# FifthEpoch/longcat-video-tta

Measured on AMD Instinct MI355X. Metric: denoised latent frames/sec (49x720p, 50-step CFG denoise), higher is better.
Workload: dtype bf16; 1 GPU; K3: 49x720p (13 latent frames, 46 800 tokens); DiT 48 blocks x 4096 hidden, CFG 4.0, 50-step flow-match Euler, no conditioning frames; depth=48, parallelism=dp1

## Files before the change

### longcat-video-tta_amd/csrc/elementwise.hip

```cpp
#include "lcv_common.h"

#define ROWNORM_MAXCH 8

template <int MODE>
__global__ __launch_bounds__(256) void rownorm_fwd_kernel(
    const bf16_t* __restrict__ x, const float* __restrict__ p_add, const float* __restrict__ p_mul,
    bf16_t* __restrict__ y, int64_t rows, int C, int64_t S, int64_t mod_stride, float eps) {
  const int lane = threadIdx.x & 63;
  const int64_t row = (int64_t)blockIdx.x * 4 + (threadIdx.x >> 6);
  if (row >= rows) return;
  const bf16_t* xr = x + row * C;
  float v[ROWNORM_MAXCH][8];
  float sum = 0.f;
#pragma unroll
  for (int ch = 0; ch < ROWNORM_MAXCH; ++ch) {
    const int c = (ch * 64 + lane) * 8;
    if (c < C) {
      u16x8 raw = *reinterpret_cast<const u16x8*>(xr + c);
      unpack8(raw, v[ch]);
#pragma unroll
      for (int i = 0; i < 8; ++i) sum += v[ch][i];
    } else {
#pragma unroll
      for (int i = 0; i < 8; ++i) v[ch][i] = 0.f;
    }
  }
  const float mean = wave_sum(sum) / (float)C;
  float sq = 0.f;
#pragma unroll
  for (int ch = 0; ch < ROWNORM_MAXCH; ++ch) {
    const int c = (ch * 64 + lane) * 8;
    if (c < C) {
#pragma unroll
      for (int i = 0; i < 8; ++i) {
        const float d = v[ch][i] - mean;
        sq += d * d;
      }
    }
  }
  const float rstd = rsqrtf(wave_sum(sq) / (float)C + eps);
  const float* pa = p_add;
  const float* pm = p_mul;
  if (MODE == 0) {
    const int64_t frame = row / S;
    pa += frame * mod_stride;
    pm += frame * mod_stride;
  }
  bf16_t* yr = y + row * C;
#pragma unroll
  for (int ch = 0; ch < ROWNORM_MAXCH; ++ch) {
    const int c = (ch * 64 + lane) * 8;
    if (c < C) {
      const f32x4 a0 = *reinterpret_cast<const f32x4*>(pa + c);
      const f32x4 a1 = *reinterpret_cast<const f32x4*>(pa + c + 4);
      const f32x4 m0 = *reinterpret_cast<const f32x4*>(pm + c);
      const f32x4 m1 = *reinterpret_cast<const f32x4*>(pm + c + 4);
      float o[8];
#pragma unroll
      for (int i = 0; i < 8; ++i) {
        const float xh = (v[ch][i] - mean) * rstd;
        const float mul = (i < 4) ? m0[i] : m1[i - 4];
        const float add = (i < 4) ? a0[i] : a1[i - 4];
        o[i] = (MODE == 0) ? (xh * (mul + 1.0f) + add) : (xh * mul + add);
      }
      *reinterpret_cast<u16x8*>(yr + c) = pack8(o);
    }
  }
}

extern "C" int lcv_adaln_modulate_fwd(const void* x, const float* mod, void* y, int64_t B, int64_t T,
                                      int64_t S, int64_t C, int64_t mod_stride, int64_t shift_off,
                                      int64_t scale_off, float eps, void* stream) {
  LCV_CHECK_ARG(x && mod && y, "adaln_modulate_fwd: null pointer");
  LCV_CHECK_ARG(C > 0 && C % 8 == 0 && C <= 4096, "adaln_modulate_fwd: C=%ld must be a multiple of 8 and <= 4096", (long)C);
  LCV_CHECK_ARG(B > 0 && T > 0 && S > 0, "adaln_modulate_fwd: bad sizes");
  LCV_CHECK_ARG(shift_off % 4 == 0 && scale_off % 4 == 0 && mod_stride % 4 == 0, "adaln_modulate_fwd: offsets must be 16-byte aligned");
  const int64_t rows = B * T * S;
  const unsigned grid = (unsigned)((rows + 3) / 4);
  hipLaunchKernelGGL(rownorm_fwd_kernel<0>, dim3(grid), dim3(256), 0, (hipStream_t)stream,
                     (const bf16_t*)x, mod + shift_off, mod + scale_off, (bf16_t*)y, rows, (int)C, S,
                     mod_stride, eps);
  LCV_LAUNCH_CHECK("adaln_modulate_fwd");
  return LCV_OK;
}

extern "C" int lcv_layernorm_affine_fwd(const void* x, const float* w, const float* b, void* y,
                                        int64_t rows, int64_t C, float eps, void* stream) {
  LCV_CHECK_ARG(x && w && b && y, "layernorm_affine_fwd: null pointer");
  LCV_CHECK_ARG(C > 0 && C % 8 == 0 && C <= 4096, "layernorm_affine_fwd: C=%ld must be a multiple of 8 and <= 4096", (long)C);
  if (rows == 0) return LCV_OK;
  const unsigned grid = (unsigned)((rows + 3) / 4);
  hipLaunchKernelGGL(rownorm_fwd_kernel<1>, dim3(grid), dim3(256), 0, (hipStream_t)stream,
                     (const bf16_t*)x, b, w, (bf16_t*)y, rows, (int)C, (int64_t)1, (int64_t)0, eps);
  LCV_LAUNCH_CHECK("layernorm_affine_fwd");
  return LCV_OK;
}

__global__ __launch_bounds__(256) void gate_residual_fwd_kernel(
    const bf16_t* __restrict__ x, const bf16_t* __restrict__ y, const float* __restrict__ gate,
    bf16_t* __restrict__ out, int64_t n_packets, int cpk , int64_t S, int64_t mod_stride) {
  for (int64_t p = (int64_t)blockIdx.x * blockDim.x + threadIdx.x; p < n_packets;
       p += (int64_t)gridDim.x * blockDim.x) {
    const int64_t row = p / cpk;
    const int c = (int)(p - row * cpk) * 8;
    float xf[8], yf[8], o[8];
    unpack8(*reinterpret_cast<const u16x8*>(x + p * 8), xf);
    unpack8(*reinterpret_cast<const u16x8*>(y + p * 8), yf);
    if (gate) {
      const float* g = gate + (row / S) * mod_stride + c;
      const f32x4 g0 = *reinterpret_cast<const f32x4*>(g);
      const f32x4 g1 = *reinterpret_cast<const f32x4*>(g + 4);
#pragma unroll
      for (int i = 0; i < 8; ++i) o[i] = xf[i] + ((i < 4) ? g0[i] : g1[i - 4]) * yf[i];
    } else {
#pragma unroll
      for (int i = 0; i < 8; ++i) o[i] = xf[i] + yf[i];
    }
    *reinterpret_cast<u16x8*>(out + p * 8) = pack8(o);
  }
}

extern "C" int lcv_gate_residual_fwd(const void* x, const void* y, const float* mod, void* out,
                                     int64_t B, int64_t T, int64_t S, int64_t C, int64_t mod_stride,
                                     int64_t gate_off, void* stream) {
  LCV_CHECK_ARG(x && y && out, "gate_residual_fwd: null pointer");
  LCV_CHECK_ARG(C > 0 && C % 8 == 0, "gate_residual_fwd: C must be a multiple of 8");
// ... 473 lines not shown
```

### longcat-video-tta_amd/csrc/lib.hip

```cpp
#include "lcv_common.h"
#include <mutex>
#include <stdlib.h>
#include <string.h>

static thread_local char g_err[512] = "";

void lcv_set_error(const char* fmt, ...) {
  va_list ap;
  va_start(ap, fmt);
  vsnprintf(g_err, sizeof(g_err), fmt, ap);
  va_end(ap);
}

extern "C" int lcv_version(void) { return 11; }

extern "C" const char* lcv_last_error(void) { return g_err; }

extern "C" int lcv_device_check(void) {
  int dev = 0;
  if (hipGetDevice(&dev) != hipSuccess) {
    lcv_set_error("device_check: no HIP device");
    return LCV_EDEVICE;
  }
  hipDeviceProp_t prop;
  if (hipGetDeviceProperties(&prop, dev) != hipSuccess) {
    lcv_set_error("device_check: hipGetDeviceProperties failed");
    return LCV_EDEVICE;
  }
  if (strncmp(prop.gcnArchName, "gfx950", 6) != 0) {
    lcv_set_error("device_check: device is %s, this library is built for gfx950 only", prop.gcnArchName);
    return LCV_EDEVICE;
  }
  return LCV_OK;
}

namespace {
struct Knob { const char* name; char value[32]; bool set; };
Knob g_knobs[] = {
    {"LCV_GEMM_TILE"}, {"LCV_GEMM_GROUP_M"}, {"LCV_GEMM_FAST_EPI"}, {"LCV_GEMM_SPLITK_TAIL"},
    {"LCV_CONV_8P"}, {"LCV_CONV_N192"}, {"LCV_CONV_ROWS"}, {"LCV_CONV_ROWS_GRID"}, {"LCV_CONV_ROWS_ORDER"},
    {"LCV_ATTN_FWD_W64"}, {"LCV_ATTN_XCD"},
    {"LCV_ATTN_BWD_VAR"}, {"LCV_ATTN_BWD_DKV_WAVES"}, {"LCV_ATTN_BWD_DQ_WAVES"}, {"LCV_ATTN_BWD_PIPE"}, {"LCV_ATTN_BWD_STAGGER"},
    {"LCV_ATTN_BWD_XCD"},
};
std::mutex g_knob_mutex;
bool g_knobs_read = false;
void knobs_read_locked() {
// ... 36 lines not shown
```

### longcat-video-tta_amd/lcv_hip/autograd_ops.py

```python
import weakref
from typing import List, Optional

import torch

from . import ops
from .lib import (LCV_EPI_GELU_TANH, LCV_EPI_NONE, LCV_EPI_SWIGLU, LcvError)

BF16 = torch.bfloat16
F32 = torch.float32

_EPI = {None: LCV_EPI_NONE, "gelu_tanh": LCV_EPI_GELU_TANH}


def _needs_grad(*ts) -> bool:
    return torch.is_grad_enabled() and any(t is not None and t.requires_grad for t in ts)


_WT_CACHE = {}


def transposed_weight(w: torch.Tensor) -> torch.Tensor:
    key = id(w)
    ent = _WT_CACHE.get(key)
    if ent is not None and ent[0]() is w and ent[1] == w._version and ent[2].data_ptr() != 0:
# ... 457 lines not shown
    @staticmethod
    def backward(ctx, do):
        q_raw, kv_raw, qn, kn, o, wq, wk, *lses = ctx.saved_tensors
        seqlens, scale, eps = ctx.args
        want_dw = wq.requires_grad or wk.requires_grad
        B, N, H, D = q_raw.shape
        L = kv_raw.shape[1]
        do = do.contiguous()
        dqn = torch.empty_like(qn)
        dkv = torch.zeros((1, L, 2, H, D), dtype=BF16, device=q_raw.device)
        off = 0
        for b in range(B):
            Lb = int(seqlens[b])
            ops.attention_bwd(qn[b:b + 1], kn[:, off:off + Lb], kv_raw[:, off:off + Lb, 1], o[b:b + 1], do[b:b + 1],
                              lses[b], dqn[b:b + 1], dkv[:, off:off + Lb, 0], dkv[:, off:off + Lb, 1], scale,
                              accumulate_kv=False)
            off += Lb
        dq_raw = torch.empty_like(q_raw)
        dwq = torch.zeros(D, dtype=torch.float32, device=q_raw.device) if want_dw else None
        dwk = torch.zeros(D, dtype=torch.float32, device=q_raw.device) if want_dw else None
        ops.qknorm_rope_bwd(q_raw, None, dqn, None, dq_raw, None, wq, wk, None, 0, eps, dwq=dwq)
        dkv_raw = torch.empty_like(kv_raw)
        ops.qknorm_rope_bwd(None, kv_raw[:, :, 0], None, dkv[:, :, 0], None, dkv_raw[:, :, 0], wq, wk, None, 0, eps, dwk=dwk)
        dkv_raw[:, :, 1].copy_(dkv[:, :, 1])
        return (dq_raw, dkv_raw, dwq.to(wq.dtype) if (want_dw and wq.requires_grad) else None,
                dwk.to(wk.dtype) if (want_dw and wk.requires_grad) else None, None, None, None)


def cross_attention(q, kv, wq, wk, seqlens: List[int], scale, eps):
    if _needs_grad(q, kv, wq, wk):
        return _CrossAttentionFn.apply(q, kv, wq, wk, seqlens, scale, eps)
    B, N, H, D = q.shape
    k, v = kv[:, :, 0], kv[:, :, 1]
    ops.qknorm_rope(q, None, None, q, None, None, wq, wk, None, 0, eps)
    ops.qknorm_rope(None, k, None, None, k, None, wq, wk, None, 0, eps)
    o = torch.empty_like(q)
    off = 0
    for b in range(B):
        Lb = int(seqlens[b])
        ops.attention(q[b:b + 1], k[:, off:off + Lb], v[:, off:off + Lb], scale, out=o[b:b + 1])
        off += Lb
    return o


class _GeluTanhFn(torch.autograd.Function):
    @staticmethod
    def forward(ctx, x):
        ctx.save_for_backward(x)
        return ops.gelu_tanh(x)

    @staticmethod
    def backward(ctx, dy):
        (x,) = ctx.saved_tensors
        return ops.gelu_tanh_bwd(x, (dy if dy.dtype == BF16 else dy.to(BF16)).contiguous())


def gelu_tanh(x: torch.Tensor) -> torch.Tensor:
    if _needs_grad(x):
        return _GeluTanhFn.apply(x)
    return ops.gelu_tanh(x)


class _SwiGLUFn(torch.autograd.Function):
    @staticmethod
    def forward(ctx, g, u):
        ctx.save_for_backward(g, u)
# ... 98 lines not shown
```

### longcat-video-tta_amd/lcv_hip/build.py

```python
import os
import subprocess
import sys
from concurrent.futures import ThreadPoolExecutor
from pathlib import Path

PKG_DIR = Path(__file__).resolve().parent
CSRC = PKG_DIR.parent / "csrc"
INCLUDE = PKG_DIR.parents[1] / "include"
BUILD = CSRC / "build"
LIB = PKG_DIR / "liblcv_hip.so"
HIPCC = os.environ.get("HIPCC", "/opt/rocm/bin/hipcc")
FLAGS = ["--offload-arch=gfx950", "-O3", "-fPIC", "-std=c++17", "-Wno-unused-value",
         "-fno-gpu-rdc", "-I", str(INCLUDE)]


def _newest_header():
    hs = list(CSRC.glob("*.h")) + list(INCLUDE.glob("*.h"))
    return max(h.stat().st_mtime for h in hs)


_ATTN_FLAGS = ["-fno-honor-nans", "-mno-amdgpu-ieee", "-fno-slp-vectorize"]
EXTRA = {"attn_fwd.hip": _ATTN_FLAGS, "attn_fwd_pipe.hip": _ATTN_FLAGS, "attn_bwd_dq2.hip": _ATTN_FLAGS, "attn_bwd_dkv2.hip": _ATTN_FLAGS,
         "attn_fwd_w64.hip": _ATTN_FLAGS,
         "optim_master.hip": ["-ffp-contract=off"], "optim_moments8.hip": ["-ffp-contract=off"],
         "optim_accum.hip": ["-ffp-contract=off"], "optim_anchor.hip": ["-ffp-contract=off"],
         "optim_ema.hip": ["-ffp-contract=off"], "step_cache.hip": ["-ffp-contract=off"],
         "solver_step.hip": ["-ffp-contract=off"]}


def _compile(src: Path, hdr_mtime: float) -> Path:
    obj = BUILD / (src.stem + ".o")
    if obj.exists() and obj.stat().st_mtime > max(src.stat().st_mtime, hdr_mtime):
        return obj
    cmd = [HIPCC, *FLAGS, *EXTRA.get(src.name, []), "-c", str(src), "-o", str(obj)]
    r = subprocess.run(cmd, capture_output=True, text=True)
    if r.returncode != 0:
        raise RuntimeError(f"hipcc failed for {src.name}:\n{r.stdout}\n{r.stderr}")
    if r.stderr.strip():
        sys.stderr.write(r.stderr)
    return obj


def build(verbose: bool = False) -> Path:
    BUILD.mkdir(exist_ok=True)
    srcs = sorted(CSRC.glob("*.hip"))
    if not srcs:
        raise RuntimeError(f"no HIP sources under {CSRC}")
    hdr = _newest_header()
    with ThreadPoolExecutor(max_workers=min(6, len(srcs))) as ex:
        objs = list(ex.map(lambda s: _compile(s, hdr), srcs))
    if LIB.exists() and all(LIB.stat().st_mtime > o.stat().st_mtime for o in objs):
        return LIB
    cmd = [HIPCC, "--offload-arch=gfx950", "-shared", "-fPIC", "-o", str(LIB), *map(str, objs)]
    r = subprocess.run(cmd, capture_output=True, text=True)
    if r.returncode != 0:
        raise RuntimeError(f"link failed:\n{r.stdout}\n{r.stderr}")
# ... 8 lines not shown
```

### longcat-video-tta_amd/lcv_hip/lib.py

```python
import ctypes
import os
from ctypes import c_char_p, c_double, c_float, c_int, c_int64, c_uint64, c_void_p
from pathlib import Path

_LIB_PATH = Path(__file__).resolve().parent / "liblcv_hip.so"

P, I64, F32, I, F64, U64 = c_void_p, c_int64, c_float, c_int, c_double, c_uint64

_SIGNATURES = {
    "lcv_device_check": [],
    "lcv_adaln_modulate_fwd": [P, P, P, I64, I64, I64, I64, I64, I64, I64, F32, P],
    "lcv_adaln_modulate_bwd": [P, P, P, P, P, I64, I64, I64, I64, I64, I64, I64, F32, P, P],
    "lcv_layernorm_affine_fwd": [P, P, P, P, I64, I64, F32, P],
    "lcv_layernorm_affine_bwd": [P, P, P, P, P, P, I64, I64, F32, P, P],
    "lcv_gate_residual_fwd": [P, P, P, P, I64, I64, I64, I64, I64, I64, P],
    "lcv_gate_residual_bwd": [P, P, P, P, P, I64, I64, I64, I64, I64, I64, P],
    "lcv_qknorm_rope_fwd": [P, P, P, P, P, P, P, P, P, I64, I64, I64, I64, I64, I64, I64, I64, I64, I64, F32, F32, P],
    "lcv_qknorm_rope_bwd": [P, P, P, P, P, P, P, P, P, I64, I64, I64, I64, I64, I64, I64, I64, I64, I64, I64, I64, F32, F32, P, P, I64, P],
    "lcv_attn_fwd": [P, P, P, P, P, I64, I64, I64, I64] + [I64] * 12 + [F32, P],
    "lcv_attn_bwd": [P, P, P, P, P, P, P, P, P, P, I, I64, I64, I64, I64] + [I64] * 21 + [F32, P],
    "lcv_gemm_nt": [P, P, P, P, P, P, I64, I64, I64, I64, I64, I64, I64, I64, I64, I, I, P, P, I64, I64, I64, P],
    "lcv_gemm_set_workspace": [P, I64],
    "lcv_linear_f32_smallm": [P, P, P, P, I64, I64, I64, I, P],
    "lcv_lora_down": [P, P, P, I64, I64, I64, I64, I64, F32, P],
# ... 69 lines not shown
    "lcv_moments8_encode": [P, P, P, P, P, I64, P],
    "lcv_moments8_decode": [P, P, P, P, P, I64, P],
}

_SIGNATURES_ACCUM = {
    "lcv_grad_accumulate": [P, P, I64, I64, F64, P],
    "lcv_master_sgd_step_g32": [P, P, I64, I64, P, F64, F64, P],
    "lcv_master_adamw_step_g32": [P, P, I64, I64, P, F64, F64, F64, F64, F64, I64, P],
}

_SIGNATURES_ANCHOR = {
    "lcv_master_sgd_step_anchor": [P, P, P, I64, I64, P, F64, F64, I, P],
    "lcv_master_adamw_step_anchor": [P, P, P, I64, I64, P, F64, F64, F64, F64, F64, I64, I, P],
    "lcv_master_adamw8_step_anchor": [P, P, P, P, I64, I64, P, F64, F64, F64, F64, F64, I64, P],
    "lcv_master_drift_sumsq": [P, P, P, I64, I64, P, I64, P, P],
}

_SIGNATURES_EMA = {
    "lcv_master_ema_load": [P, P, P, I64, I64, P],
    "lcv_master_ema_update": [P, P, P, I64, I64, F64, P],
    "lcv_master_ema_swap": [P, P, P, I64, I64, P],
}

_SIGNATURES_STEPCACHE = {
    "lcv_stepcache_diff": [P, P, P, P, I64, I64, F32, P, I64, P, P],
    "lcv_stepcache_store": [P, P, P, I64, P],
    "lcv_stepcache_apply": [P, P, P, I64, P],
}

_SIGNATURES_SOLVER = {
    "lcv_cfg_lms_step": [P, P, P, P, P, P, P, I64, I64, F32, F32, F32, F32, I, I, I, P],
}

LCV_EPI_NONE, LCV_EPI_SWIGLU, LCV_EPI_GATE_RESIDUAL, LCV_EPI_GELU_TANH, LCV_EPI_SILU = 0, 1, 2, 3, 4


class LcvError(RuntimeError):
    code = None

    @property
    def fatal(self) -> bool:
        return self.code in (-2, -3)


_lib = None


def lib_path() -> Path:
    return _LIB_PATH


def load():
    global _lib
    if _lib is not None:
        return _lib
    if not _LIB_PATH.exists():
        raise LcvError(
            f"{_LIB_PATH} is missing: build it with `python __graft_entry__.py` (hipcc, gfx950). "
            "There is no fallback path.")
    import torch
    lib = ctypes.CDLL(str(_LIB_PATH), mode=os.RTLD_NOW | getattr(os, "RTLD_LOCAL", 0))
    lib.lcv_version.restype = c_int
    lib.lcv_version.argtypes = []
    lib.lcv_last_error.restype = c_char_p
    lib.lcv_last_error.argtypes = []
    lib.lcv_attn_fwd_last_kernel.restype = c_char_p
    lib.lcv_attn_fwd_last_kernel.argtypes = []
    lib.lcv_knobs_list.restype = c_char_p
    lib.lcv_knobs_list.argtypes = []
    lib.lcv_knobs_reload.restype = c_int
    lib.lcv_knobs_reload.argtypes = []
    lib.lcv_conv3d_last_kernel.restype = c_char_p
    lib.lcv_conv3d_last_kernel.argtypes = []
    lib.lcv_tn_skinny_ws_bytes.restype = c_int64
    lib.lcv_tn_skinny_ws_bytes.argtypes = [I64, I64, I64]
    lib.lcv_attn_bwd_ws_floats.restype = c_int64
    lib.lcv_attn_bwd_ws_floats.argtypes = [I64, I64, I64, I64]
    lib.lcv_lpips_ws_bytes.restype = c_int64
    lib.lcv_lpips_ws_bytes.argtypes = [I64, I64, I64]
    lib.lcv_det_ws_bytes.restype = c_int64
    lib.lcv_det_ws_bytes.argtypes = [I, I64, I64, I64]
    lib.lcv_tn_skinny_dropout_ws_bytes.restype = c_int64
    lib.lcv_tn_skinny_dropout_ws_bytes.argtypes = [I64, I64, I64]
    for name, args in (list(_SIGNATURES.items()) + list(_SIGNATURES_LPIPS.items()) + list(_SIGNATURES_DET.items())
                       + list(_SIGNATURES_LORA.items()) + list(_SIGNATURES_MASTER.items()) + list(_SIGNATURES_MOMENTS8.items())
                       + list(_SIGNATURES_ACCUM.items()) + list(_SIGNATURES_ANCHOR.items()) + list(_SIGNATURES_EMA.items())
                       + list(_SIGNATURES_STEPCACHE.items()) + list(_SIGNATURES_SOLVER.items())):
        fn = getattr(lib, name, None)
        if fn is None:
            continue
        fn.restype = c_int
        fn.argtypes = args
    _lib = lib
    return lib


def reload_knobs() -> int:
    return load().lcv_knobs_reload()


def set_knob(name: str, value) -> None:
    if value is None:
        os.environ.pop(name, None)
    else:
        os.environ[name] = str(value)
    if _lib is not None:
        _lib.lcv_knobs_reload()


def call(name: str, *args):
    lib = load()
    fn = getattr(lib, name)
    rc = fn(*args)
    if rc != 0:
        msg = lib.lcv_last_error()
        err = LcvError(f"{name} failed ({rc}): {msg.decode() if msg else ''}")
        err.code = rc
        raise err
```

### longcat-video-tta_amd/lcv_hip/ops.py

```python
import os
from typing import Optional, Tuple

import torch

from . import lib as _lib
from .lib import (LCV_EPI_GATE_RESIDUAL, LCV_EPI_GELU_TANH, LCV_EPI_NONE, LCV_EPI_SILU, LCV_EPI_SWIGLU,
                  call)

BF16 = torch.bfloat16
F32 = torch.float32
PROFILE = None
PROFILE_BWD = None


_DETERMINISTIC = os.environ.get("LCV_DETERMINISTIC", "") == "1"


def set_deterministic(flag: bool) -> None:
    global _DETERMINISTIC
    _DETERMINISTIC = bool(flag)


def is_deterministic() -> bool:
    return _DETERMINISTIC
# ... 100 lines not shown
         ko.stride(0), ko.stride(1), pos_off, eps, q_scale, _stream())


LOG2E = 1.4426950408889634
LN2 = 0.6931471805599453


def log2_qscale(scale: float) -> float:
    return scale * LOG2E


def attention(q: torch.Tensor, k: torch.Tensor, v: torch.Tensor, scale: float,
              out: Optional[torch.Tensor] = None, need_lse: bool = False) -> Tuple[torch.Tensor, Optional[torch.Tensor]]:
    for t, nme in ((q, "q"), (k, "k"), (v, "v")):
        _req(t, BF16, "attention." + nme)
        if t.shape[-1] != 128 or t.stride(-1) != 1:
            raise _lib.LcvError("attention: head_dim must be 128 and contiguous")
    B, Nq, H, D = q.shape
    Nk = k.shape[1]
    if out is None:
        out = torch.empty((B, Nq, H, D), dtype=BF16, device=q.device)
    lse = torch.empty((B, H, Nq), dtype=F32, device=q.device) if need_lse else None
    if PROFILE is not None:
        ev0 = torch.cuda.Event(enable_timing=True); ev1 = torch.cuda.Event(enable_timing=True)
        ev0.record()
    call("lcv_attn_fwd", _ptr(q), _ptr(k), _ptr(v), _ptr(out), _ptr(lse), B, H, Nq, Nk,
         q.stride(0), q.stride(1), q.stride(2), k.stride(0), k.stride(1), k.stride(2),
         v.stride(0), v.stride(1), v.stride(2), out.stride(0), out.stride(1), out.stride(2),
         float(scale), _stream())
    if PROFILE is not None:
        ev1.record()
        PROFILE.append((ev0, ev1, 4.0 * B * H * Nq * Nk * D, Nq, Nk, _lib.load().lcv_attn_fwd_last_kernel().decode()))
    return out, lse


_GEMM_WS = {}
GEMM_WS_BYTES = 256 << 20


def _ensure_gemm_workspace(device: torch.device) -> None:
    idx = device.index if device.index is not None else torch.cuda.current_device()
    if idx not in _GEMM_WS:
        if _GEMM_WS:
            raise _lib.LcvError(
                f"gemm_nt on cuda:{idx}, but this process already bound the library's split-K workspace to cuda:"
                f"{next(iter(_GEMM_WS))}: the build runs one process per GPU (torch.distributed), a second device in the "
                "same process would write its partial sums into the first device's memory")
        ws = torch.empty(GEMM_WS_BYTES, dtype=torch.uint8, device=device)
        call("lcv_gemm_set_workspace", _ptr(ws), GEMM_WS_BYTES)
        _GEMM_WS[idx] = ws


PARAM_EPOCH = 0


def gemm_nt(a: torch.Tensor, w: torch.Tensor, bias: Optional[torch.Tensor] = None, *,
            a2: Optional[torch.Tensor] = None, w2: Optional[torch.Tensor] = None,
            epilogue: int = LCV_EPI_NONE, out_f32: bool = False, resid: Optional[torch.Tensor] = None,
            mod: Optional[torch.Tensor] = None, gate_idx: int = 0, rows_per_frame: int = 1,
            out: Optional[torch.Tensor] = None, swiglu_aux: Optional[torch.Tensor] = None) -> torch.Tensor:
    _req(a, BF16, "gemm_nt.a"); _req(w, BF16, "gemm_nt.w")
    if a.shape[0] >= 2048:
        _ensure_gemm_workspace(a.device)
    if a.dim() != 2 or w.dim() != 2 or a.stride(1) != 1 or w.stride(1) != 1:
        raise _lib.LcvError("gemm_nt: a and w must be 2-D with contiguous rows")
    M, K = a.shape
# ... 1175 lines not shown
```

Before: 0.06140 latent frames/s.

## Add fused text cross-attention kernel and stage modulation params in LDS for rownorm

Adds a dedicated cross-attention kernel for short text keys (at most 256) that fuses the query RMS-norm with its weight into the attention pass and keeps all K/V tiles resident in LDS, using a persistent grid sized from occupancy. The separate q-norm pass and the generic attention launch go away on the default path. Separately, the rownorm/adaLN kernel now processes runs of rows per block within a frame and loads the shift/scale vectors once into shared memory instead of once per row. The risks are reduced parallelism for small frames and a numerics difference from double bf16 rounding in the fused q-norm.

```diff
diff --git a/include/lcv_hip_xattn.h b/include/lcv_hip_xattn.h
--- /dev/null
+++ b/include/lcv_hip_xattn.h
@@ -0,0 +1,19 @@
+#ifndef LCV_HIP_XATTN_H
+#define LCV_HIP_XATTN_H
+
+#include <stdint.h>
+#include "lcv_hip.h"
+
+#ifdef __cplusplus
+extern "C" {
+#endif
+
+int lcv_xattn_text_fwd(const void* q, const void* k, const void* v, void* o, const void* wq, const int64_t* kv_len, int64_t B,
+                       int64_t H, int64_t Nq, int64_t q_sb, int64_t q_sn, int64_t q_sh, int64_t k_sn, int64_t k_sh,
+                       int64_t v_sn, int64_t v_sh, int64_t o_sb, int64_t o_sn, int64_t o_sh, float scale, float eps,
+                       int64_t max_workgroups, void* stream);
+
+#ifdef __cplusplus
+}
+#endif
+#endif
diff --git a/longcat-video-tta_amd/csrc/elementwise.hip b/longcat-video-tta_amd/csrc/elementwise.hip
--- a/longcat-video-tta_amd/csrc/elementwise.hip
+++ b/longcat-video-tta_amd/csrc/elementwise.hip
@@ -1,71 +1,101 @@
 #include "lcv_common.h"
 
 #define ROWNORM_MAXCH 8
+#ifndef ROWNORM_RUN
+#define ROWNORM_RUN 32
+#endif
 
 template <int MODE>
 __global__ __launch_bounds__(256) void rownorm_fwd_kernel(
     const bf16_t* __restrict__ x, const float* __restrict__ p_add, const float* __restrict__ p_mul,
-    bf16_t* __restrict__ y, int64_t rows, int C, int64_t S, int64_t mod_stride, float eps) {
+    bf16_t* __restrict__ y, int64_t rows, int C, int64_t S, int64_t mod_stride, int runs_per_frame, float eps) {
+  __shared__ f32x4 s_add[ROWNORM_MAXCH * 2 * 64];
+  __shared__ f32x4 s_mul[ROWNORM_MAXCH * 2 * 64];
   const int lane = threadIdx.x & 63;
-  const int64_t row = (int64_t)blockIdx.x * 4 + (threadIdx.x >> 6);
-  if (row >= rows) return;
-  const bf16_t* xr = x + row * C;
-  float v[ROWNORM_MAXCH][8];
-  float sum = 0.f;
-#pragma unroll
-  for (int ch = 0; ch < ROWNORM_MAXCH; ++ch) {
-    const int c = (ch * 64 + lane) * 8;
-    if (c < C) {
-      u16x8 raw = *reinterpret_cast<const u16x8*>(xr + c);
-      unpack8(raw, v[ch]);
-#pragma unroll
-      for (int i = 0; i < 8; ++i) sum += v[ch][i];
-    } else {
-#pragma unroll
-      for (int i = 0; i < 8; ++i) v[ch][i] = 0.f;
-    }
-  }
-  const float mean = wave_sum(sum) / (float)C;
-  float sq = 0.f;
-#pragma unroll
-  for (int ch = 0; ch < ROWNORM_MAXCH; ++ch) {
-    const int c = (ch * 64 + lane) * 8;
-    if (c < C) {
-#pragma unroll
-      for (int i = 0; i < 8; ++i) {
-        const float d = v[ch][i] - mean;
-        sq += d * d;
+  const int64_t frame = (int64_t)blockIdx.x / runs_per_frame;
+  const int64_t run = (int64_t)blockIdx.x - frame * runs_per_frame;
+  const int64_t row0 = frame * S + run * ROWNORM_RUN;
+  int64_t row_end = row0 + ROWNORM_RUN;
+  if (row_end > frame * S + S) row_end = frame * S + S;
+  if (row_end > rows) row_end = rows;
+  {
+    const float* pa = p_add;
+    const float* pm = p_mul;
+    if (MODE == 0) {
+      pa += frame * mod_stride;
+      pm += frame * mod_stride;
+    }
+    for (int j = threadIdx.x; j < C / 4; j += 256) {
+      const int g = j >> 1;
+      const int slot = (((g >> 6) * 2 + (j & 1)) << 6) + (g & 63);
+      s_add[slot] = *reinterpret_cast<const f32x4*>(pa + 4 * j);
+      s_mul[slot] = *reinterpret_cast<const f32x4*>(pm + 4 * j);
+    }
+  }
+  __syncthreads();
+  for (int64_t row = row0 + (threadIdx.x >> 6); row < row_end; row += 4) {
+    const bf16_t* xr = x + row * C;
+    float v[ROWNORM_MAXCH][8];
+    float sum = 0.f;
+#pragma unroll
+    for (int ch = 0; ch < ROWNORM_MAXCH; ++ch) {
+      const int c = (ch * 64 + lane) * 8;
+      if (c < C) {
+        u16x8 raw = *reinterpret_cast<const u16x8*>(xr + c);
+        unpack8(raw, v[ch]);
+#pragma unroll
+        for (int i = 0; i < 8; ++i) sum += v[ch][i];
+      } else {
+#pragma unroll
+        for (int i = 0; i < 8; ++i) v[ch][i] = 0.f;
       }
     }
-  }
-  const float rstd = rsqrtf(wave_sum(sq) / (float)C + eps);
-  const float* pa = p_add;
-  const float* pm = p_mul;
-  if (MODE == 0) {
-    const int64_t frame = row / S;
-    pa += frame * mod_stride;
-    pm += frame * mod_stride;
-  }
-  bf16_t* yr = y + row * C;
-#pragma unroll
-  for (int ch = 0; ch < ROWNORM_MAXCH; ++ch) {
-    const int c = (ch * 64 + lane) * 8;
-    if (c < C) {
-      const f32x4 a0 = *reinterpret_cast<const f32x4*>(pa + c);
-      const f32x4 a1 = *reinterpret_cast<const f32x4*>(pa + c + 4);
-      const f32x4 m0 = *reinterpret_cast<const f32x4*>(pm + c);
-      const f32x4 m1 = *reinterpret_cast<const f32x4*>(pm + c + 4);
-      float o[8];
-#pragma unroll
-      for (int i = 0; i < 8; ++i) {
-        const float xh = (v[ch][i] - mean) * rstd;
-        const float mul = (i < 4) ? m0[i] : m1[i - 4];
-        const float add = (i < 4) ? a0[i] : a1[i - 4];
-        o[i] = (MODE == 0) ? (xh * (mul + 1.0f) + add) : (xh * mul + add);
+    const float mean = wave_sum(sum) / (float)C;
+    float sq = 0.f;
+#pragma unroll
+    for (int ch = 0; ch < ROWNORM_MAXCH; ++ch) {
+      const int c = (ch * 64 + lane) * 8;
+      if (c < C) {
+#pragma unroll
+        for (int i = 0; i < 8; ++i) {
+          const float d = v[ch][i] - mean;
+          sq += d * d;
+        }
       }
-      *reinterpret_cast<u16x8*>(yr + c) = pack8(o);
-    }
-  }
+    }
+    const float rstd = rsqrtf(wave_sum(sq) / (float)C + eps);
+    bf16_t* yr = y + row * C;
+#pragma unroll
+    for (int ch = 0; ch < ROWNORM_MAXCH; ++ch) {
+      const int c = (ch * 64 + lane) * 8;
+      if (c < C) {
+        const f32x4 a0 = s_add[(2 * ch) * 64 + lane];
+        const f32x4 a1 = s_add[(2 * ch + 1) * 64 + lane];
+        const f32x4 m0 = s_mul[(2 * ch) * 64 + lane];
+        const f32x4 m1 = s_mul[(2 * ch + 1) * 64 + lane];
+        float o[8];
+#pragma unroll
+        for (int i = 0; i < 8; ++i) {
+          const float xh = (v[ch][i] - mean) * rstd;
+          const float mul = (i < 4) ? m0[i] : m1[i - 4];
+          const float add = (i < 4) ? a0[i] : a1[i - 4];
+          o[i] = (MODE == 0) ? (xh * (mul + 1.0f) + add) : (xh * mul + add);
+        }
+        *reinterpret_cast<u16x8*>(yr + c) = pack8(o);
+      }
+    }
+  }
+}
+
+template <int MODE>
+static int rownorm_launch(const char* name, const bf16_t* x, const float* p_add, const float* p_mul, bf16_t* y, int64_t rows,
+                          int64_t C, int64_t S, int64_t mod_stride, float eps, hipStream_t stream) {
+  const int64_t frames = (rows + S - 1) / S;
+  const int64_t rpf = (S + ROWNORM_RUN - 1) / ROWNORM_RUN;
+  LCV_CHECK_ARG(frames * rpf <= 0x7fffffff, "%s: too many rows", name);
+  hipLaunchKernelGGL(rownorm_fwd_kernel<MODE>, dim3((unsigned)(frames * rpf)), dim3(256), 0, stream, x, p_add, p_mul, y, rows,
+                     (int)C, S, mod_stride, (int)rpf, eps);
+  return LCV_OK;
 }
 
 extern "C" int lcv_adaln_modulate_fwd(const void* x, const float* mod, void* y, int64_t B, int64_t T,
@@ -75,11 +105,9 @@
   LCV_CHECK_ARG(C > 0 && C % 8 == 0 && C <= 4096, "adaln_modulate_fwd: C=%ld must be a multiple of 8 and <= 4096", (long)C);
   LCV_CHECK_ARG(B > 0 && T > 0 && S > 0, "adaln_modulate_fwd: bad sizes");
   LCV_CHECK_ARG(shift_off % 4 == 0 && scale_off % 4 == 0 && mod_stride % 4 == 0, "adaln_modulate_fwd: offsets must be 16-byte aligned");
-  const int64_t rows = B * T * S;
-  const unsigned grid = (unsigned)((rows + 3) / 4);
-  hipLaunchKernelGGL(rownorm_fwd_kernel<0>, dim3(grid), dim3(256), 0, (hipStream_t)stream,
-                     (const bf16_t*)x, mod + shift_off, mod + scale_off, (bf16_t*)y, rows, (int)C, S,
-                     mod_stride, eps);
+  const int rc = rownorm_launch<0>("adaln_modulate_fwd", (const bf16_t*)x, mod + shift_off, mod + scale_off, (bf16_t*)y,
+                                   B * T * S, C, S, mod_stride, eps, (hipStream_t)stream);
+  if (rc != LCV_OK) return rc;
   LCV_LAUNCH_CHECK("adaln_modulate_fwd");
   return LCV_OK;
 }
@@ -89,9 +117,10 @@
   LCV_CHECK_ARG(x && w && b && y, "layernorm_affine_fwd: null pointer");
   LCV_CHECK_ARG(C > 0 && C % 8 == 0 && C <= 4096, "layernorm_affine_fwd: C=%ld must be a multiple of 8 and <= 4096", (long)C);
   if (rows == 0) return LCV_OK;
-  const unsigned grid = (unsigned)((rows + 3) / 4);
-  hipLaunchKernelGGL(rownorm_fwd_kernel<1>, dim3(grid), dim3(256), 0, (hipStream_t)stream,
-                     (const bf16_t*)x, b, w, (bf16_t*)y, rows, (int)C, (int64_t)1, (int64_t)0, eps);
+  LCV_CHECK_ARG(rows > 0, "layernorm_affine_fwd: bad sizes");
+  const int rc = rownorm_launch<1>("layernorm_affine_fwd", (const bf16_t*)x, b, w, (bf16_t*)y, rows, C, rows, 0, eps,
+                                   (hipStream_t)stream);
+  if (rc != LCV_OK) return rc;
   LCV_LAUNCH_CHECK("layernorm_affine_fwd");
   return LCV_OK;
 }
diff --git a/longcat-video-tta_amd/csrc/lib.hip b/longcat-video-tta_amd/csrc/lib.hip
--- a/longcat-video-tta_amd/csrc/lib.hip
+++ b/longcat-video-tta_amd/csrc/lib.hip
@@ -12,7 +12,7 @@
   va_end(ap);
 }
 
-extern "C" int lcv_version(void) { return 11; }
+extern "C" int lcv_version(void) { return 12; }
 
 extern "C" const char* lcv_last_error(void) { return g_err; }
 
diff --git a/longcat-video-tta_amd/csrc/xattn_text.hip b/longcat-video-tta_amd/csrc/xattn_text.hip
--- /dev/null
+++ b/longcat-video-tta_amd/csrc/xattn_text.hip
@@ -0,0 +1,368 @@
+#include "attn_common.h"
+#include "../../include/lcv_hip_xattn.h"
+#include <type_traits>
+
+#define XT_MAX_B 8
+#define XT_MAX_L 256
+#define XT_TILE_BYTES (64 * 256)
+#define XT_OSTAGE_BYTES (8 * 2048)
+
+struct XattnTextParams {
+  const bf16_t* q;
+  const bf16_t* k;
+  const bf16_t* v;
+  bf16_t* o;
+  const bf16_t* wq;
+  int64_t Nq, q_sb, q_sn, q_sh, k_sn, k_sh, v_sn, v_sh, o_sb, o_sn, o_sh;
+  int H;
+  int gx;
+  int per;
+  int cpp;
+  int nitems;
+  int grid;
+  int lds_o_off;
+  int o16;
+  float scale_log2e, eps;
+  int kv_len[XT_MAX_B], kv_off[XT_MAX_B];
+};
+
+__device__ __forceinline__ float xt_rsqrtf(float x) {
+  const bool small = 0x1p-126f > x;
+  const float y = __builtin_amdgcn_rsqf(small ? x * 0x1p+24f : x);
+  return small ? y * 0x1p+12f : y;
+}
+
+__device__ __forceinline__ float xt_lo(unsigned u) { return __builtin_bit_cast(float, u << 16); }
+__device__ __forceinline__ float xt_hi(unsigned u) { return __builtin_bit_cast(float, u & 0xffff0000u); }
+__device__ __forceinline__ void xt_unpack8(const u16x8& v, float (&f)[8]) {
+  const u32x4 u = __builtin_bit_cast(u32x4, v);
+#pragma unroll
+  for (int j = 0; j < 4; ++j) { f[2 * j] = xt_lo(u[j]); f[2 * j + 1] = xt_hi(u[j]); }
+}
+__device__ __forceinline__ unsigned xt_pack2(float lo, float hi) {
+  unsigned y;
+  asm("v_cvt_pk_bf16_f32 %0, %1, %2" : "=v"(y) : "v"(lo), "v"(hi));
+  return y;
+}
+
+__global__ __launch_bounds__(512) void xattn_text_fwd_kernel(const XattnTextParams p) {
+  extern __shared__ __attribute__((aligned(16))) unsigned char smem[];
+  lds_u8* lds = (lds_u8*)smem;
+  __shared__ f32x4 s_wq[32];
+
+  const int tid = (int)__builtin_amdgcn_workitem_id_x();
+  const int lane = tid & 63;
+  const int wave = __builtin_amdgcn_readfirstlane(tid >> 6);
+  const int r = lane & 31, h = lane >> 5;
+
+  if (tid < 32) {
+    const u16x4 w = *reinterpret_cast<const u16x4*>(p.wq + 4 * tid);
+    s_wq[tid] = f32x4{bf2f(w[0]), bf2f(w[1]), bf2f(w[2]), bf2f(w[3])};
+  }
+
+  const int kf = attn_swz(r);
+  const int k_row_off = 256 * r;
+  const int q4 = (lane >> 2) & 3, p4 = lane & 3, g1 = (lane >> 4) & 1;
+  int v_base[2], v_low[2];
+#pragma unroll
+  for (int half = 0; half < 2; ++half) {
+    v_base[half] = 256 * (4 * h + 8 * half + q4) + 8 * (p4 & 1);
+    v_low[half] = (2 * g1 + (p4 >> 1)) ^ (h + 2 * half);
+  }
+
+  auto load_q = [&](u16x8 (&raw)[8], int64_t b, int head, int blk) {
+    int64_t qrow = (int64_t)blk * 256 + wave * 32 + r;
+    if (qrow > p.Nq - 1) qrow = p.Nq - 1;
+    const bf16_t* qp = p.q + b * p.q_sb + qrow * p.q_sn + (int64_t)head * p.q_sh + 8 * h;
+#pragma unroll
+    for (int ks = 0; ks < 8; ++ks) raw[ks] = *reinterpret_cast<const u16x8*>(qp + 16 * ks);
+  };
+
+  for (int item = (int)__builtin_amdgcn_workgroup_id_x(); item < p.nitems; item += p.grid) {
+    const int pair = item / p.cpp, chunk = item - pair * p.cpp;
+    const int bi = pair / p.H, head = pair - bi * p.H;
+    const int64_t b = bi;
+    int L = p.kv_len[0], off = p.kv_off[0];
+#pragma unroll
+    for (int i = 1; i < XT_MAX_B; ++i) {
+      if (bi == i) { L = p.kv_len[i]; off = p.kv_off[i]; }
+    }
+    const int nt = (L + 63) >> 6;
+    const int blk0 = chunk * p.per;
+    const int blk1 = (blk0 + p.per < p.gx) ? blk0 + p.per : p.gx;
+
+    u16x8 qraw[8];
+    load_q(qraw, b, head, blk0);
+
+    {
+      const bf16_t* kbase = p.k + (int64_t)off * p.k_sn + (int64_t)head * p.k_sh;
+      const bf16_t* vbase = p.v + (int64_t)off * p.v_sn + (int64_t)head * p.v_sh;
+      u32x4 kreg[4][2], vreg[4][2];
+#pragma unroll
+      for (int t = 0; t < 4; ++t)
+#pragma unroll
+        for (int i = 0; i < 2; ++i) {
+          const int c = tid + 512 * i;
+          int row = 64 * t + (c >> 4);
+          if (row > L - 1) row = L - 1;
+          kreg[t][i] = *reinterpret_cast<const u32x4*>(kbase + (int64_t)row * p.k_sn + (c & 15) * 8);
+          vreg[t][i] = *reinterpret_cast<const u32x4*>(vbase + (int64_t)row * p.v_sn + (c & 15) * 8);
+        }
+      __syncthreads();
+#pragma unroll
+      for (int t = 0; t < 4; ++t) {
+        if (t < nt) {
+#pragma unroll
+          for (int i = 0; i < 2; ++i) {
+            const int c = tid + 512 * i;
+            const int o = 2 * XT_TILE_BYTES * t + attn_tile_off(c >> 4, c & 15);
+            *reinterpret_cast<AS3 u32x4*>(lds + o) = kreg[t][i];
+            *reinterpret_cast<AS3 u32x4*>(lds + XT_TILE_BYTES + o) = vreg[t][i];
+          }
+        }
+      }
+      __syncthreads();
+    }
+
+    for (int blk = blk0; blk < blk1; ++blk) {
+      bf16x8 qf[8];
+      {
+        float ssq[8];
+#pragma unroll
+        for (int ks = 0; ks < 8; ++ks) {
+          float f[8];
+          xt_unpack8(qraw[ks], f);
+          float ss = 0.f;
+#pragma unroll
+          for (int i = 0; i < 8; ++i) ss += f[i] * f[i];
+          ssq[ks] = ss;
+        }
+        float l8[4], l4[2];
+#pragma unroll
+        for (int j = 0; j < 4; ++j) l8[j] = ssq[j] + ssq[j + 4];
+#pragma unroll
+        for (int j = 0; j < 2; ++j) l4[j] = l8[j] + l8[j + 2];
+        float ss = l4[0] + l4[1];
+        ss = half_sum(ss);
+        const float rn = xt_rsqrtf(ss * (1.0f / 128.0f) + p.eps);
+#pragma unroll
+        for (int ks = 0; ks < 8; ++ks) {
+          float f[8];
+          xt_unpack8(qraw[ks], f);
+          const f32x4 w0 = s_wq[2 * (2 * ks + h)], w1 = s_wq[2 * (2 * ks + h) + 1];
+          u32x4 packed;
+#pragma unroll
+          for (int j = 0; j < 4; ++j) {
+            const unsigned once = xt_pack2(f[2 * j] * rn, f[2 * j + 1] * rn);
+            const float wl = (j < 2) ? w0[2 * j] : w1[2 * j - 4], wh = (j < 2) ? w0[2 * j + 1] : w1[2 * j - 3];
+            packed[j] = xt_pack2(xt_lo(once) * wl, xt_hi(once) * wh);
+          }
+          qf[ks] = __builtin_bit_cast(bf16x8, packed);
+        }
+      }
+      if (blk + 1 < blk1) load_q(qraw, b, head, blk + 1);
+
+      f32x16 oacc[4];
+      float m_run = -INFINITY;
+      float l_run = 0.f;
+
+      auto tile_body = [&](const int t, auto first_c) {
+        constexpr bool FIRST = decltype(first_c)::value;
+        const lds_u8* kb = lds + 2 * XT_TILE_BYTES * t;
+        const lds_u8* vb = kb + XT_TILE_BYTES;
+
+        f32x16 s0, s1;
+#pragma unroll
+        for (int e = 0; e < 16; ++e) { s0[e] = 0.f; s1[e] = 0.f; }
+#pragma unroll
+        for (int ks = 0; ks < 8; ++ks) {
+          const int co = 16 * ((2 * ks + h) ^ kf);
+          const bf16x8 a0 = *reinterpret_cast<const AS3 bf16x8*>(kb + k_row_off + co);
+          const bf16x8 a1 = *reinterpret_cast<const AS3 bf16x8*>(kb + 32 * 256 + k_row_off + co);
+          s0 = __builtin_amdgcn_mfma_f32_32x32x16_bf16(a0, qf[ks], s0, 0, 0, 0);
+          s1 = __builtin_amdgcn_mfma_f32_32x32x16_bf16(a1, qf[ks], s1, 0, 0, 0);
+        }
+
+        if (t == nt - 1 && (L & 63)) {
+          int valid = L - t * 64;
+          asm volatile("" : "+s"(valid));
+#pragma unroll
+          for (int e = 0; e < 16; ++e) {
+            const int key = (e & 3) + 8 * (e >> 2) + 4 * h;
+            if (key >= valid) s0[e] = -INFINITY;
+            if (key + 32 >= valid) s1[e] = -INFINITY;
+          }
+        }
+
+        float mxa = s0[0], mxb = s1[0];
+#pragma unroll
+        for (int e = 1; e < 16; ++e) {
+          mxa = fmaxf(mxa, s0[e]);
+          mxb = fmaxf(mxb, s1[e]);
+        }
+        float mx = fmaxf(mxa, mxb);
+        mx = half_max(mx);
+        float psum = 0.f;
+        if constexpr (FIRST) {
+          m_run = mx;
+        } else if (__builtin_amdgcn_ballot_w64((mx - m_run) * p.scale_log2e > ATTN_RESCALE_THR) != 0ull) {
+          const float m_new = fmaxf(m_run, mx);
+          const float alpha = __builtin_amdgcn_exp2f((m_run - m_new) * p.scale_log2e);
+          m_run = m_new;
+          l_run *= alpha;
+#pragma unroll
+          for (int d = 0; d < 4; ++d)
+#pragma unroll
+            for (int e = 0; e < 16; ++e) oacc[d][e] *= alpha;
+        }
+        const float mc = m_run * p.scale_log2e;
+#pragma unroll
+        for (int e = 0; e < 16; ++e) {
+          s0[e] = __builtin_amdgcn_exp2f(s0[e] * p.scale_log2e - mc);
+          s1[e] = __builtin_amdgcn_exp2f(s1[e] * p.scale_log2e - mc);
+          psum += s0[e] + s1[e];
+        }
+        l_run += psum;
+
+        bf16x8 pb[4];
+#pragma unroll
+        for (int j = 0; j < 8; ++j) {
+          pb[0][j] = (__bf16)s0[j];
+          pb[1][j] = (__bf16)s0[8 + j];
+          pb[2][j] = (__bf16)s1[j];
+          pb[3][j] = (__bf16)s1[8 + j];
+        }
+
+#pragma unroll
+        for (int kk = 0; kk < 4; ++kk) {
+#pragma unroll
+          for (int d = 0; d < 4; ++d) {
+            const int dx = 64 * (d ^ q4);
+            const s16x4 lo = __builtin_amdgcn_ds_read_tr16_b64_v4i16(
+                (AS3 s16x4*)(vb + v_base[0] + 4096 * kk + dx + 16 * v_low[0]));
+            const s16x4 hi = __builtin_amdgcn_ds_read_tr16_b64_v4i16(
+                (AS3 s16x4*)(vb + v_base[1] + 4096 * kk + dx + 16 * v_low[1]));
+            const bf16x8 vf = __builtin_bit_cast(bf16x8, __builtin_shufflevector(lo, hi, 0, 1, 2, 3, 4, 5, 6, 7));
+            if (FIRST && kk == 0) {
+              f32x16 zero;
+#pragma unroll
+              for (int e = 0; e < 16; ++e) zero[e] = 0.f;
+              oacc[d] = __builtin_amdgcn_mfma_f32_32x32x16_bf16(vf, pb[kk], zero, 0, 0, 0);
+            } else {
+              oacc[d] = __builtin_amdgcn_mfma_f32_32x32x16_bf16(vf, pb[kk], oacc[d], 0, 0, 0);
+            }
+          }
+        }
+      };
+      {
+        using Y = std::true_type;
+        using N = std::false_type;
+        tile_body(0, Y{});
+        for (int t = 1; t < nt; ++t) tile_body(t, N{});
+      }
+
+      const float l_tot = half_sum(l_run);
+      const float inv = 1.0f / l_tot;
+      lds_u8* ost = lds + p.lds_o_off + wave * 2048;
+      const int64_t orow0 = (int64_t)blk * 256 + wave * 32;
+      bf16_t* obase = p.o + b * p.o_sb + (int64_t)head * p.o_sh + 8 * (lane & 3);
+#pragma unroll
+      for (int d = 0; d < 4; ++d) {
+#pragma unroll
+        for (int i = 0; i < 4; ++i) {
+          u16x4 pk;
+#pragma unroll
+          for (int e = 0; e < 4; ++e) pk[e] = f2bf(oacc[d][4 * i + e] * inv);
+          *reinterpret_cast<AS3 u16x4*>(ost + 64 * r + 16 * (i ^ ((r >> 1) & 3)) + 8 * h) = pk;
+        }
+        __builtin_amdgcn_wave_barrier();
+#pragma unroll
+        for (int j = 0; j < 2; ++j) {
+          const int row = 16 * j + (lane >> 2);
+          const u32x4 val = *reinterpret_cast<const AS3 u32x4*>(ost + 64 * row + 16 * ((lane & 3) ^ ((row >> 1) & 3)));
+          if (orow0 + row < p.Nq) {
+            bf16_t* op = obase + (orow0 + row) * p.o_sn + 32 * d;
+            if (p.o16) {
+              *reinterpret_cast<u32x4*>(op) = val;
+            } else {
+              *reinterpret_cast<u32x2*>(op) = u32x2{val[0], val[1]};
+              *reinterpret_cast<u32x2*>(op + 4) = u32x2{val[2], val[3]};
+            }
+          }
+        }
+        __builtin_amdgcn_wave_barrier();
+      }
+    }
+  }
+}
+
+extern "C" int lcv_xattn_text_fwd(const void* q, const void* k, const void* v, void* o, const void* wq,
+                                  const int64_t* kv_len, int64_t B, int64_t H, int64_t Nq, int64_t q_sb, int64_t q_sn,
+                                  int64_t q_sh, int64_t k_sn, int64_t k_sh, int64_t v_sn, int64_t v_sh, int64_t o_sb,
+                                  int64_t o_sn, int64_t o_sh, float scale, float eps, int64_t max_workgroups, void* stream) {
+  LCV_CHECK_ARG(q && k && v && o && wq && kv_len, "xattn_text_fwd: null pointer");
+  LCV_CHECK_ARG(B >= 1 && B <= XT_MAX_B, "xattn_text_fwd: B=%ld must be 1..%d", (long)B, XT_MAX_B);
+  LCV_CHECK_ARG(H >= 1 && H <= 65535, "xattn_text_fwd: H=%ld must be 1..65535", (long)H);
+  LCV_CHECK_ARG(Nq >= 0 && Nq <= ((int64_t)1 << 38), "xattn_text_fwd: bad Nq");
+  LCV_CHECK_ARG(scale > 0.f, "xattn_text_fwd: scale must be positive");
+  LCV_CHECK_ARG(max_workgroups >= 0,"xattn_text_fwd: max_workgroups must be >= 0 (0 = the default grid)");
+  XattnTextParams p = {};
+  int64_t off = 0, lmax = 0;
+  for (int64_t b = 0; b < B; ++b) {
+    LCV_CHECK_ARG(kv_len[b] >= 1 && kv_len[b] <= XT_MAX_L, "xattn_text_fwd: kv_len[%ld]=%ld must be 1..%d", (long)b,
+                  (long)kv_len[b], XT_MAX_L);
+    p.kv_len[b] = (int)kv_len[b];
+    p.kv_off[b] = (int)off;
+    off += kv_len[b];
+    if (kv_len[b] > lmax) lmax = kv_len[b];
+  }
+  LCV_CHECK_ARG(q_sn % 8 == 0 && k_sn % 8 == 0 && v_sn % 8 == 0 && q_sh % 8 == 0 && k_sh % 8 == 0 && v_sh % 8 == 0 &&
+                    q_sb % 8 == 0,
+                "xattn_text_fwd: q/k/v strides must be multiples of 8 elements");
+  LCV_CHECK_ARG(o_sn % 4 == 0 && o_sh % 4 == 0 && o_sb % 4 == 0, "xattn_text_fwd: o strides must be multiples of 4 elements");
+  LCV_CHECK_ARG(((uintptr_t)q % 16 == 0) && ((uintptr_t)k % 16 == 0) && ((uintptr_t)v % 16 == 0) && ((uintptr_t)o % 8 == 0) &&
+                    ((uintptr_t)wq % 16 == 0),
+                "xattn_text_fwd: pointers must be 16-byte aligned");
+  if (Nq == 0) return LCV_OK;
+
+  const int64_t gx = (Nq + 255) / 256;
+  const size_t lds_tiles = (size_t)((lmax + 63) / 64) * 2 * XT_TILE_BYTES;
+  const size_t lds = lds_tiles + XT_OSTAGE_BYTES;
+  ATTN_RAISE_LDS_ONCE("xattn_text_fwd", attn_raise_lds((const void*)xattn_text_fwd_kernel, 4 * 2 * XT_TILE_BYTES + XT_OSTAGE_BYTES));
+  int64_t wgs = max_workgroups;
+  if (wgs == 0) {
+    static int resident[5] = {0, 0, 0, 0, 0};
+    const int nt = (int)((lmax + 63) / 64);
+    if (resident[nt] == 0) {
+      int dev = 0, cus = 0, per_cu = 0;
+      if (hipGetDevice(&dev) != hipSuccess ||
+          hipDeviceGetAttribute(&cus, hipDeviceAttributeMultiprocessorCount, dev) != hipSuccess ||
+          hipOccupancyMaxActiveBlocksPerMultiprocessor(&per_cu, xattn_text_fwd_kernel, 512, lds) != hipSuccess || cus <= 0 ||
+          per_cu <= 0) {
+        lcv_set_error("xattn_text_fwd: cannot read the device's CU count or the kernel's occupancy");
+        return LCV_EDEVICE;
+      }
+      resident[nt] = cus * per_cu;
+    }
+    wgs = resident[nt];
+  }
+  int64_t cpp = wgs / (B * H);
+  if (cpp < 1) cpp = 1;
+  if (cpp > gx) cpp = gx;
+  const int64_t per = (gx + cpp - 1) / cpp;
+  cpp = (gx + per - 1) / per;
+  const int64_t nitems = B * H * cpp;
+  LCV_CHECK_ARG(nitems <= 0x7fffffff, "xattn_text_fwd: too many work items");
+  const int64_t grid = nitems < wgs ? nitems : wgs;
+
+  p.q = (const bf16_t*)q; p.k = (const bf16_t*)k; p.v = (const bf16_t*)v; p.o = (bf16_t*)o; p.wq = (const bf16_t*)wq;
+  p.Nq = Nq; p.q_sb = q_sb; p.q_sn = q_sn; p.q_sh = q_sh; p.k_sn = k_sn; p.k_sh = k_sh; p.v_sn = v_sn; p.v_sh = v_sh;
+  p.o_sb = o_sb; p.o_sn = o_sn; p.o_sh = o_sh;
+  p.H = (int)H; p.gx = (int)gx; p.per = (int)per; p.cpp = (int)cpp; p.nitems = (int)nitems; p.grid = (int)grid;
+  p.lds_o_off = (int)lds_tiles;
+  p.o16 = ((uintptr_t)o % 16 == 0 && o_sn % 8 == 0 && o_sh % 8 == 0 && o_sb % 8 == 0) ? 1 : 0;
+  p.scale_log2e = scale * 1.4426950408889634f; p.eps = eps;
+  hipLaunchKernelGGL(xattn_text_fwd_kernel, dim3((unsigned)grid), dim3(512), lds, (hipStream_t)stream, p);
+  LCV_LAUNCH_CHECK("xattn_text_fwd");
+  return LCV_OK;
+}
diff --git a/longcat-video-tta_amd/lcv_hip/autograd_ops.py b/longcat-video-tta_amd/lcv_hip/autograd_ops.py
--- a/longcat-video-tta_amd/lcv_hip/autograd_ops.py
+++ b/longcat-video-tta_amd/lcv_hip/autograd_ops.py
@@ -513,6 +513,9 @@
         return _CrossAttentionFn.apply(q, kv, wq, wk, seqlens, scale, eps)
     B, N, H, D = q.shape
     k, v = kv[:, :, 0], kv[:, :, 1]
+    if ops.XATTN_TEXT and B <= ops.XATTN_TEXT_MAX_B and all(1 <= int(s) <= ops.XATTN_TEXT_MAX_L for s in seqlens):
+        ops.qknorm_rope(None, k, None, None, k, None, wq, wk, None, 0, eps)
+        return ops.cross_attention_text(q, k, v, wq, seqlens, scale, eps)
     ops.qknorm_rope(q, None, None, q, None, None, wq, wk, None, 0, eps)
     ops.qknorm_rope(None, k, None, None, k, None, wq, wk, None, 0, eps)
     o = torch.empty_like(q)
diff --git a/longcat-video-tta_amd/lcv_hip/build.py b/longcat-video-tta_amd/lcv_hip/build.py
--- a/longcat-video-tta_amd/lcv_hip/build.py
+++ b/longcat-video-tta_amd/lcv_hip/build.py
@@ -22,6 +22,7 @@
 _ATTN_FLAGS = ["-fno-honor-nans", "-mno-amdgpu-ieee", "-fno-slp-vectorize"]
 EXTRA = {"attn_fwd.hip": _ATTN_FLAGS, "attn_fwd_pipe.hip": _ATTN_FLAGS, "attn_bwd_dq2.hip": _ATTN_FLAGS, "attn_bwd_dkv2.hip": _ATTN_FLAGS,
          "attn_fwd_w64.hip": _ATTN_FLAGS,
+         "xattn_text.hip": _ATTN_FLAGS,
          "optim_master.hip": ["-ffp-contract=off"], "optim_moments8.hip": ["-ffp-contract=off"],
          "optim_accum.hip": ["-ffp-contract=off"], "optim_anchor.hip": ["-ffp-contract=off"],
          "optim_ema.hip": ["-ffp-contract=off"], "step_cache.hip": ["-ffp-contract=off"],
diff --git a/longcat-video-tta_amd/lcv_hip/lib.py b/longcat-video-tta_amd/lcv_hip/lib.py
--- a/longcat-video-tta_amd/lcv_hip/lib.py
+++ b/longcat-video-tta_amd/lcv_hip/lib.py
@@ -125,7 +125,11 @@
     "lcv_cfg_lms_step": [P, P, P, P, P, P, P, I64, I64, F32, F32, F32, F32, I, I, I, P],
 }
 
-LCV_EPI_NONE, LCV_EPI_SWIGLU, LCV_EPI_GATE_RESIDUAL, LCV_EPI_GELU_TANH, LCV_EPI_SILU = 0, 1, 2, 3, 4
+_SIGNATURES_XATTN = {
+    "lcv_xattn_text_fwd": [P, P, P, P, P, P, I64, I64, I64] + [I64] * 10 + [F32, F32, I64, P],
+}
+
+LCV_EPI_NONE, LCV_EPI_SWIGLU,LCV_EPI_GATE_RESIDUAL, LCV_EPI_GELU_TANH, LCV_EPI_SILU = 0, 1, 2, 3, 4
 
 
 class LcvError(RuntimeError):
@@ -178,7 +182,8 @@
     for name, args in (list(_SIGNATURES.items()) + list(_SIGNATURES_LPIPS.items()) + list(_SIGNATURES_DET.items())
                        + list(_SIGNATURES_LORA.items()) + list(_SIGNATURES_MASTER.items()) + list(_SIGNATURES_MOMENTS8.items())
                        + list(_SIGNATURES_ACCUM.items()) + list(_SIGNATURES_ANCHOR.items()) + list(_SIGNATURES_EMA.items())
-                       + list(_SIGNATURES_STEPCACHE.items()) + list(_SIGNATURES_SOLVER.items())):
+                       + list(_SIGNATURES_STEPCACHE.items()) + list(_SIGNATURES_SOLVER.items())
+                       + list(_SIGNATURES_XATTN.items())):
         fn = getattr(lib, name, None)
         if fn is None:
             continue
diff --git a/longcat-video-tta_amd/lcv_hip/ops.py b/longcat-video-tta_amd/lcv_hip/ops.py
--- a/longcat-video-tta_amd/lcv_hip/ops.py
+++ b/longcat-video-tta_amd/lcv_hip/ops.py
@@ -156,6 +156,34 @@
         ev1.record()
         PROFILE.append((ev0, ev1, 4.0 * B * H * Nq * Nk * D, Nq, Nk, _lib.load().lcv_attn_fwd_last_kernel().decode()))
     return out, lse
+
+
+XATTN_TEXT = True
+XATTN_TEXT_MAX_B = 8
+XATTN_TEXT_MAX_L = 256
+
+
+def cross_attention_text(q: torch.Tensor, k: torch.Tensor, v: torch.Tensor, wq: torch.Tensor, seqlens, scale: float,
+                         eps: float = 1e-6, out: Optional[torch.Tensor] = None, max_workgroups: int = 0) -> torch.Tensor:
+    for t, nme in ((q, "q"), (k, "k"), (v, "v")):
+        _req(t, BF16, "cross_attention_text." + nme)
+        if t.dim() != 4 or t.shape[-1] != 128 or t.stride(-1) != 1:
+            raise _lib.LcvError("cross_attention_text: tensors are [.., .., H, 128] with head_dim contiguous")
+    _req(wq, BF16, "cross_attention_text.wq")
+    B, Nq, H, D = q.shape
+    lens = [int(s) for s in seqlens]
+    if len(lens) != B or k.shape[0] != 1 or v.shape[0] != 1 or k.shape[1] < sum(lens) or v.shape[1] < sum(lens) \
+            or k.shape[2] != H or v.shape[2] != H or wq.numel() != D or not wq.is_contiguous():
+        raise _lib.LcvError("cross_attention_text: one length per batch row, k / v [1, >= sum(seqlens), H, 128], wq [128]")
+    if out is None:
+        out = torch.empty((B, Nq, H, D), dtype=BF16, device=q.device)
+    elif out.dtype != BF16 or out.shape != q.shape or out.stride(-1) != 1:
+        raise _lib.LcvError("cross_attention_text: out must be bf16 of q's shape with head_dim contiguous")
+    kv_len =(_lib.I64 * B)(*lens)
+    call("lcv_xattn_text_fwd", _ptr(q), _ptr(k), _ptr(v), _ptr(out), _ptr(wq), kv_len, B, H, Nq,
+         q.stride(0), q.stride(1), q.stride(2), k.stride(1), k.stride(2), v.stride(1), v.stride(2),
+         out.stride(0), out.stride(1), out.stride(2), float(scale), float(eps), int(max_workgroups), _stream())
+    return out
 
 
 _GEMM_WS = {}
```

New measurement: 0.06185 latent frames/s (median of 6 runs). No clear change (+0.7%).
